# mklarqvist/libflagstats

Measured on AMD Instinct MI355X. Metric: Gflags/s + achieved HBM GB/s vs roofline, 8 GiB uint16, 1/2/4/8 MI355X, higher is better.
Workload: dtype u16; 1 GPU; 8 GiB uniform-random uint16 FLAG array (4294967296 flags) per GPU, device-resident, K1 flagstat_count accumulating into the 32 counters (atomic epilogue, one launch); flags_per_gpu=4294967296, global_flags=4294967296, parallelism=shard1, kernel_variant=71, grid_blocks=256

## Files before the change

libflagstats_amd/csrc/flagstat_capi.hip:

```cpp
#include <hip/hip_runtime.h>

#include <cstdio>
#include <cstdlib>
#include <cstring>

#include "../../include/libflagstats_hip_probe.h"
#include "flagstat_engine.h"
#include "flagstat_kernels.h"

using fsint::DeviceGuard;
using fsint::Engine;
using fsint::fail_hip;
using fsint::fail_text;

struct FLAGSTATS_hip_ctx {
    Engine* engine;
};

namespace {

#define HIP_TRY(expr)                                      \
    do {                                                   \
        hipError_t e_ = (expr);                            \
        if (e_ != hipSuccess) return fail_hip(#expr, e_);  \
// ... 121 lines not shown
        if (!fsk_variant_supported(static_cast<int>(value)))
            return fail_text("this build carries K1 schedules 9, 25 and 71 only (the sweeps' losers need make TUNING=1)");
        k.variant = static_cast<int>(value);
    } else if (!std::strcmp(key, "fuse")) {
        if (value > 1) return fail_text("fuse must be 0 or 1");
        if (value && !fsk_tuning_build())
            return fail_text("the ticket-fused finalise lost to K1 + K2 and to the atomic epilogue; it is carried by the tuning build only (make TUNING=1)");
        k.fuse = static_cast<int>(value);
    } else if (!std::strcmp(key, "anatomy")) {
        if (!fsk_tuning_build()) return fail_text("anatomy is a tuning-build knob (make TUNING=1)");
        fsk_set_anatomy(static_cast<int>(value));
    } else if (!std::strcmp(key, "epilogue")) {
        if (value > 1) return fail_text("epilogue must be 0 (partials + K2) or 1 (atomic adds from K1)");
        k.epilogue = static_cast<int>(value);
    } else if (!std::strcmp(key, "small_flags")) {
        k.small_flags = value;
    } else if (!std::strcmp(key, "small_bar")) {
        if (value > 1) return fail_text("small_bar must be 0 or 1");
        k.small_bar = static_cast<int>(value);
    } else if (!std::strcmp(key, "poll")) {
        if (value > 1) return fail_text("poll must be 0 or 1");
        k.poll = static_cast<int>(value);
    } else if (!std::strcmp(key, "epoch_stagger")) {
        if (value > 1) return fail_text("epoch_stagger must be 0 or 1");
        k.epoch_stagger = static_cast<int>(value);
        fsk_set_epoch_stagger(k.epoch_stagger.load());
    } else if (!std::strcmp(key, "group_min_grid")) {
        if (value > 0xFFFFFFFFull) return fail_text("group_min_grid must fit 32 bits");
        k.group_min_grid = static_cast<uint32_t>(value);
        fsk_set_group_min_grid(k.group_min_grid.load());
    } else if (!std::strcmp(key, "group_max_steps")) {
        k.group_max_steps = value;
        fsk_set_group_max_steps(value);
    } else if (!std::strcmp(key, "dyn_lg_queues")) {
        if (value > 4) return fail_text("dyn_lg_queues must be 0..4");
        k.dyn_lgq = static_cast<uint32_t>(value);
        if (fsk_tuning_build()) fsk_set_dyn_queues(k.dyn_lgq.load());
    } else if (!std::strcmp(key, "dyn_first_pct") || !std::strcmp(key, "dyn_div") || !std::strcmp(key, "dyn_cmax") ||
               !std::strcmp(key, "dyn_min_steps")) {
        std::atomic<uint32_t>& slot = key[4] == 'f' ? k.dyn_first_pct : key[4] == 'd' ? k.dyn_div : key[4] == 'c' ? k.dyn_cmax : k.dyn_min_steps;
        if ((key[4] == 'f' && value > 100) || (key[4] == 'd' && (value < 1 || value > 64)) || (key[4] == 'c' && (value < 1 || value > 65535)) ||
            value > 0xFFFFFFFFull)
            return fail_text("dyn_first_pct 0..100, dyn_div 1..64, dyn_cmax 1..65535");
        slot = static_cast<uint32_t>(value);
        if (fsk_tuning_build()) fsk_set_dyn(k.dyn_first_pct.load(), k.dyn_div.load(), k.dyn_cmax.load(), k.dyn_min_steps.load());
    } else if (!std::strcmp(key, "chunk_flags")) {
        if (value < 8) return fail_text("chunk_flags must be >= 8");
        k.chunk_flags = value;
    } else if (!std::strcmp(key, "on_error")) {
        if (value > 1) return fail_text("on_error must be 0 (return) or 1 (abort)");
        k.on_error = static_cast<int>(value);
    } else if (!std::strcmp(key, "fence_free_events")) {
        if (value > 1) return fail_text("fence_free_events must be 0 or 1");
        k.fence_free_events = static_cast<int>(value);
    } else if (!std::strcmp(key, "lz4_decoder")) {
        if (value > 2) return fail_text("lz4_decoder must be 0 (host threads), 1 (GPU) or 2 (by file size)");
        k.lz4_decoder = static_cast<int>(value);
    } else if (!std::strcmp(key, "zstd_decoder")) {
        if (value > 2) return fail_text("zstd_decoder must be 0 (libzstd on host threads), 1 (GPU) or 2 (by file size)");
        k.zstd_decoder = static_cast<int>(value);
    } else if (!std::strcmp(key, "zstd_gpu_min_bytes")) {
        k.zstd_gpu_min_bytes = value;
    } else if (!std::strcmp(key, "lz4_gpu_kernel")) {
        if (value > 1) return fail_text("lz4_gpu_kernel must be 0 (workgroup pipeline) or 1 (one wave per block)");
        k.lz4_gpu_kernel = static_cast<int>(value);
    } else if (!std::strcmp(key, "lz4_gpu_min_bytes")) {
        k.lz4_gpu_min_bytes = value;
    } else if (!std::strcmp(key, "staged_min_flags")) {
        k.staged_min_flags = value;
    } else if (!std::strcmp(key, "lz4_gpu_keep_bytes")) {
        k.lz4_gpu_keep_bytes = value;
    } else if (!std::strcmp(key, "numa")) {
        if (value > 1) return fail_text("numa must be 0 or 1");
        k.numa = static_cast<int>(value);
    } else {
        return fail_text("unknown key");
    }
    return 0;
}

uint64_t FLAGSTATS_hip_get(const char* key)
{
    if (fsint::process_guard(__func__)) return 0;
    if (!key) return 0;
    fsint::Knobs& k = fsint::knobs();
    if (!std::strcmp(key, "blocks_per_cu")) return k.blocks_per_cu ? k.blocks_per_cu.load() : 1;
    if (!std::strcmp(key, "variant")) return static_cast<uint64_t>(k.variant.load());
    if (!std::strcmp(key, "chunk_flags")) return k.chunk_flags.load();
    if (!std::strcmp(key, "dyn_first_pct")) return k.dyn_first_pct.load();
    if (!std::strcmp(key, "dyn_div")) return k.dyn_div.load();
    if (!std::strcmp(key, "dyn_cmax")) return k.dyn_cmax.load();
    if (!std::strcmp(key, "dyn_min_steps")) return k.dyn_min_steps.load();
    if (!std::strcmp(key, "dyn_lg_queues")) return k.dyn_lgq.load();
    if (!std::strcmp(key, "group_min_grid")) return k.group_min_grid.load();
    if (!std::strcmp(key, "group_max_steps")) return k.group_max_steps.load();
    if (!std::strcmp(key, "last_k1_two_level")) return (fsk_last_mode() >> 3) & 1;
    if (!std::strcmp(key, "small_flags")) return k.small_flags.load();
    if (!std::strcmp(key, "small_bar")) return static_cast<uint64_t>(k.small_bar.load());
    if (!std::strcmp(key, "small_in_is_device")) {
        if (fsint::default_device() < 0) return 0;
        Engine* e = fsint::default_engine();
        return e && e->small_bar_in ? 1 : 0;
    }
    if (!std::strcmp(key, "poll")) return static_cast<uint64_t>(k.poll.load());
    if (!std::strcmp(key, "epoch_stagger")) return static_cast<uint64_t>(k.epoch_stagger.load());
    if (!std::strcmp(key, "fuse")) return static_cast<uint64_t>(k.fuse.load());
    if (!std::strcmp(key, "epilogue")) return static_cast<uint64_t>(k.epilogue.load());
    if (!std::strcmp(key, "tuning_build")) return static_cast<uint64_t>(fsk_tuning_build());
    if (!std::strcmp(key, "on_error")) return static_cast<uint64_t>(k.on_error.load());
    if (!std::strcmp(key, "numa")) return static_cast<uint64_t>(k.numa.load());
    if (!std::strcmp(key, "lz4_decoder")) return static_cast<uint64_t>(k.lz4_decoder.load());
    if (!std::strcmp(key, "zstd_decoder")) return static_cast<uint64_t>(k.zstd_decoder.load());
    if (!std::strcmp(key, "zstd_gpu_min_bytes")) return k.zstd_gpu_min_bytes.load();
    if (!std::strcmp(key, "lz4_gpu_kernel")) return static_cast<uint64_t>(k.lz4_gpu_kernel.load());
    if (!std::strcmp(key, "lz4_gpu_min_bytes")) return k.lz4_gpu_min_bytes.load();
    if (!std::strcmp(key, "staged_min_flags")) return k.staged_min_flags.load();
    if (!std::strcmp(key, "staged_calls")) return k.staged_calls.load();
    if (!std::strcmp(key, "lz4_gpu_keep_bytes")) return k.lz4_gpu_keep_bytes.load();
    if (!std::strcmp(key, "lz4_gpu_kept_bytes")) {
        if (fsint::default_device() < 0) return 0;
        Engine* e = fsint::default_engine();
        if (!e) return 0;
        std::lock_guard<std::mutex> lk(e->mu);
        uint64_t held = e->lz4_cap[0] + e->lz4_cap[1];
        for (uint64_t c : e->zstd_scratch_cap) held += c;
        return held;
    }
    if (!std::strcmp(key, "user_workspaces")) {
        if (fsint::default_device() < 0) return 0;
// ... 467 lines not shown
```

libflagstats_amd/csrc/flagstat_count_core.h:

```cpp
#ifndef FLAGSTAT_COUNT_CORE_H_
#define FLAGSTAT_COUNT_CORE_H_

#include <hip/hip_runtime.h>
#include <stdint.h>

#include "flagstat_device.h"
#include "flagstat_kernels.h"

namespace fsk {

__device__ __forceinline__ void front4(uint32_t L, uint32_t H, uint32_t& T, uint32_t& selq, uint32_t& keep)
{
    const uint32_t sel1 = (L >> 1) & 0x07070707u;
    const uint32_t abc = perm(0x09091B19u, 0x09092B29u, sel1);
    const uint32_t m = __builtin_amdgcn_bitop3_b32(L, abc, 0xC4C4C4C4u, 0xE4);

    const uint32_t h1 = H >> 1;
    const uint32_t idx = and_or(h1, 0x04040404u, lshl1_or(L & 0x01010101u, H & 0x01010101u));
    keep = perm(0x050C050Cu, 0x05F60504u, idx);
    T = m & keep;

    selq = h1 & 0x03030303u;
}

// ... 161 lines not shown
        if constexpr (ATOMIC) {
            if (add) (void)__hip_atomic_fetch_add(&out[threadIdx.x], add, __ATOMIC_RELAXED, __HIP_MEMORY_SCOPE_AGENT);
        } else {
            if (mode & 1)
                out[threadIdx.x] = add;
            else if (add)
                out[threadIdx.x] += add;
        }
    }
}

__device__ __forceinline__ void grouped_epilogue(const uint64_t* tot, uint64_t* __restrict__ out, int mode, uint64_t n_flags,
                                                 uint64_t* __restrict__ block)
{
    if (threadIdx.x >= 64) return;
    const uint32_t g = blockIdx.x & 7u;
    const uint32_t members = (gridDim.x - g + 7u) >> 3;
    uint64_t* copy = block + kGroupCopyWord + 32 * g;
    uint64_t* ticket = block + kGroupTicketWord + 16 * g;
    const uint64_t add = threadIdx.x < 32 ? slot_value(tot, mode, n_flags) : 0;
    if (add) (void)__hip_atomic_fetch_add(&copy[threadIdx.x], add, __ATOMIC_RELAXED, __HIP_MEMORY_SCOPE_AGENT);
    asm volatile("s_waitcnt vmcnt(0)" ::: "memory");
    uint32_t t = 0;
    if (threadIdx.x == 0) t = static_cast<uint32_t>(__hip_atomic_fetch_add(ticket, 1ull, __ATOMIC_RELAXED, __HIP_MEMORY_SCOPE_AGENT));
    t = __builtin_amdgcn_readfirstlane(t);
    if (t != members - 1) return;
    if (threadIdx.x < 32) {
        const uint64_t v = __hip_atomic_exchange(&copy[threadIdx.x], 0ull, __ATOMIC_RELAXED, __HIP_MEMORY_SCOPE_AGENT);
        if (v) (void)__hip_atomic_fetch_add(&out[threadIdx.x], v, __ATOMIC_RELAXED, __HIP_MEMORY_SCOPE_AGENT);
    }
    if (threadIdx.x == 0) __hip_atomic_store(ticket, 0ull, __ATOMIC_RELAXED, __HIP_MEMORY_SCOPE_AGENT);
}

template <bool NT, int USTRIDE, int VPS = kVecPerStep>
__device__ __forceinline__ void load_step(uint4 (&v)[kUnroll], const uint4* __restrict__ a0, uint64_t st, uint64_t lane_off,
                                          uint64_t lo, uint64_t hi, uint64_t fast_begin, uint64_t fast_end)
{
    const uint64_t j0 = st * VPS + lane_off;
    if (st >= fast_begin && st < fast_end) {
#pragma unroll
        for (int u = 0; u < kUnroll; ++u) v[u] = load_vec<NT>(a0 + j0 + u * USTRIDE);
    } else {
#pragma unroll
        for (int u = 0; u < kUnroll; ++u) v[u] = load_guarded(a0, j0 + u * USTRIDE, lo, hi);
    }
}

}

#endif
```

libflagstats_amd/csrc/flagstat_engine.h:

```cpp
#ifndef FLAGSTAT_ENGINE_H_
#define FLAGSTAT_ENGINE_H_

#include <hip/hip_runtime.h>
#include <stdint.h>

#include <sched.h>

#include <atomic>
#include <cstdio>
#include <condition_variable>
#include <functional>
#include <list>
#include <memory>
#include <mutex>
#include <thread>
#include <utility>
#include <vector>

struct FLAGSTATS_gpu_lz4_stats;

namespace fsint {

struct Workspace {
    uint64_t* partials = nullptr;
    uint32_t grid_cap = 0;
};

struct Knobs {
    std::atomic<uint32_t> blocks_per_cu{0};
    std::atomic<int> variant{71};
    std::atomic<uint32_t> dyn_first_pct{75}, dyn_div{4}, dyn_cmax{32}, dyn_min_steps{32}, dyn_lgq{3};
    std::atomic<uint64_t> small_flags{1ull << 20};
    std::atomic<int> small_bar{1};
    std::atomic<int> poll{1};
    std::atomic<int> epoch_stagger{1};
    std::atomic<uint32_t> group_min_grid{64};
    std::atomic<uint64_t> group_max_steps{40};
    std::atomic<int> fuse{0};
    std::atomic<int> epilogue{1};
    std::atomic<uint64_t> chunk_flags{32ull << 20};
    std::atomic<int> on_error{1};
    std::atomic<int> lz4_decoder{2};
    std::atomic<int> lz4_gpu_kernel{0};
    std::atomic<uint64_t> lz4_gpu_min_bytes{64ull << 20};
    std::atomic<uint64_t> staged_min_flags{1ull << 27};
    std::atomic<uint64_t> staged_calls{0};
    std::atomic<uint64_t> lz4_gpu_keep_bytes{~0ull};
    std::atomic<int> zstd_decoder{2};
    std::atomic<uint64_t> zstd_gpu_min_bytes{64ull << 20};
    std::atomic<int> fence_free_events{0};
    std::atomic<int> numa{1};
};
Knobs& knobs();

enum { OP_FLAGSTAT = 0, OP_POSPOPCNT = 1, OP_FLAGSTAT_STORE = 2, OP_BASE_MASK = 3, OP_SUPERSET = 4, OP_HOST_OUT = 8 };

struct RegisteredHost {
    void* ptr = nullptr;
    void* map = nullptr;
    size_t map_bytes = 0;
    size_t len = 0;
    bool registered = false;
    bool refused = false;
};

class WorkerPool {
  public:
    WorkerPool() = default;
    ~WorkerPool();
    WorkerPool(const WorkerPool&) = delete;
    WorkerPool& operator=(const WorkerPool&) = delete;
    bool start(int n, std::function<void(int)> fn);
    void wait();
    int threads() const { return static_cast<int>(threads_.size()); }

  private:
    void loop(int id, uint64_t born);
    std::mutex m_;
    std::condition_variable cv_job_, cv_done_;
    std::vector<std::thread> threads_;
    std::function<void(int)> job_;
    uint64_t generation_ = 0;
    int want_ = 0, running_ = 0;
    bool stop_ = false;
};

// ... 180 lines not shown
```

libflagstats_amd/csrc/flagstat_engine.hip:

```cpp
#include "flagstat_engine.h"

#include <emmintrin.h>
#include <smmintrin.h>
#include <sys/syscall.h>
#include <pthread.h>
#include <sys/mman.h>
#include <unistd.h>

#include <cstdio>
#include <cstdlib>
#include <chrono>
#include <cstring>
#include <memory>
#include <string>
#include <thread>
#include <vector>

#include "flagstat_kernels.h"

namespace fsint {

namespace {

constexpr size_t kHostOutBytes = 1024;
// ... 28 lines not shown
        }
        if (have == 0xFFFFFFFFu) return 0;
        _mm_pause();
    }
    return 1;
}

uint64_t env_u64(const char* name, uint64_t dflt)
{
    const char* s = std::getenv(name);
    if (!s || !*s) return dflt;
    return std::strtoull(s, nullptr, 0);
}

void read_env_knobs()
{
    std::call_once(g_env_once, [] {
        g_knobs.blocks_per_cu = static_cast<uint32_t>(env_u64("FLAGSTATS_HIP_BLOCKS_PER_CU", g_knobs.blocks_per_cu));
        g_knobs.variant = static_cast<int>(env_u64("FLAGSTATS_HIP_VARIANT", static_cast<uint64_t>(g_knobs.variant)));
        g_knobs.chunk_flags = env_u64("FLAGSTATS_HIP_CHUNK_FLAGS", g_knobs.chunk_flags);
        g_knobs.dyn_first_pct = static_cast<uint32_t>(env_u64("FLAGSTATS_HIP_DYN_FIRST_PCT", g_knobs.dyn_first_pct));
        g_knobs.dyn_div = static_cast<uint32_t>(env_u64("FLAGSTATS_HIP_DYN_DIV", g_knobs.dyn_div));
        g_knobs.dyn_cmax = static_cast<uint32_t>(env_u64("FLAGSTATS_HIP_DYN_CMAX", g_knobs.dyn_cmax));
        g_knobs.dyn_min_steps = static_cast<uint32_t>(env_u64("FLAGSTATS_HIP_DYN_MIN_STEPS", g_knobs.dyn_min_steps));
        g_knobs.small_flags = env_u64("FLAGSTATS_HIP_SMALL_FLAGS", g_knobs.small_flags);
        g_knobs.small_bar = static_cast<int>(env_u64("FLAGSTATS_HIP_SMALL_BAR", static_cast<uint64_t>(g_knobs.small_bar)));
        g_knobs.poll = static_cast<int>(env_u64("FLAGSTATS_HIP_POLL", static_cast<uint64_t>(g_knobs.poll)));
        g_knobs.epoch_stagger = static_cast<int>(env_u64("FLAGSTATS_HIP_EPOCH_STAGGER", static_cast<uint64_t>(g_knobs.epoch_stagger)));
        fsk_set_epoch_stagger(g_knobs.epoch_stagger.load());
        g_knobs.group_min_grid = static_cast<uint32_t>(env_u64("FLAGSTATS_HIP_GROUP_MIN_GRID", g_knobs.group_min_grid));
        fsk_set_group_min_grid(g_knobs.group_min_grid.load());
        g_knobs.group_max_steps = env_u64("FLAGSTATS_HIP_GROUP_MAX_STEPS", g_knobs.group_max_steps);
        fsk_set_group_max_steps(g_knobs.group_max_steps.load());
        g_knobs.dyn_lgq = static_cast<uint32_t>(env_u64("FLAGSTATS_HIP_DYN_LG_QUEUES", g_knobs.dyn_lgq));
        if (fsk_tuning_build()) {
            fsk_set_dyn_queues(g_knobs.dyn_lgq.load());
            fsk_set_dyn(g_knobs.dyn_first_pct.load(), g_knobs.dyn_div.load(), g_knobs.dyn_cmax.load(), g_knobs.dyn_min_steps.load());
        }
        g_knobs.fuse = fsk_tuning_build() ? static_cast<int>(env_u64("FLAGSTATS_HIP_FUSE", static_cast<uint64_t>(g_knobs.fuse))) : 0;
        g_knobs.epilogue = static_cast<int>(env_u64("FLAGSTATS_HIP_EPILOGUE", static_cast<uint64_t>(g_knobs.epilogue)));
        g_knobs.numa = static_cast<int>(env_u64("FLAGSTATS_HIP_NUMA", static_cast<uint64_t>(g_knobs.numa)));
        g_knobs.fence_free_events = static_cast<int>(env_u64("FLAGSTATS_HIP_FENCE_FREE_EVENTS", static_cast<uint64_t>(g_knobs.fence_free_events)));
        g_knobs.lz4_decoder = static_cast<int>(env_u64("FLAGSTATS_HIP_LZ4_DECODER", static_cast<uint64_t>(g_knobs.lz4_decoder)));
        g_knobs.lz4_gpu_kernel = static_cast<int>(env_u64("FLAGSTATS_HIP_LZ4_GPU_KERNEL", static_cast<uint64_t>(g_knobs.lz4_gpu_kernel)));
        g_knobs.lz4_gpu_min_bytes = env_u64("FLAGSTATS_HIP_LZ4_GPU_MIN_BYTES", g_knobs.lz4_gpu_min_bytes);
        g_knobs.staged_min_flags = env_u64("FLAGSTATS_HIP_STAGED_MIN_FLAGS", g_knobs.staged_min_flags);
        g_knobs.zstd_decoder = static_cast<int>(env_u64("FLAGSTATS_HIP_ZSTD_DECODER", static_cast<uint64_t>(g_knobs.zstd_decoder)));
        if (g_knobs.zstd_decoder > 2) g_knobs.zstd_decoder = 2;
        g_knobs.zstd_gpu_min_bytes = env_u64("FLAGSTATS_HIP_ZSTD_GPU_MIN_BYTES", g_knobs.zstd_gpu_min_bytes);
        g_knobs.lz4_gpu_keep_bytes = env_u64("FLAGSTATS_HIP_LZ4_GPU_KEEP_BYTES", g_knobs.lz4_gpu_keep_bytes);
        const char* oe = std::getenv("FLAGSTATS_HIP_ON_ERROR");
        if (oe && *oe) g_knobs.on_error = (!std::strcmp(oe, "return") || !std::strcmp(oe, "0")) ? 0 : 1;
    });
}

#define HIP_TRY(expr)                                      \
    do {                                                   \
        hipError_t e_ = (expr);                            \
        if (e_ != hipSuccess) return fail_hip(#expr, e_);  \
    } while (0)

int numa_node_of_device(int device)
{
    char bus[64] = {0};
    if (hipDeviceGetPCIBusId(bus, sizeof bus, device) != hipSuccess) return -1;
    for (char* p = bus; *p; ++p)
// ... 232 lines not shown
        std::lock_guard<std::mutex> lk(m_);
        job_ = std::move(fn);
        want_ = n;
        running_ = n;
        ++generation_;
    }
    cv_job_.notify_all();
    return true;
}

void WorkerPool::wait()
{
    {
        std::unique_lock<std::mutex> ul(m_);
        cv_done_.wait(ul, [&] { return running_ == 0; });
        want_ = 0;
    }
    static const bool per_call = [] {
        const char* k = std::getenv("FLAGSTATS_HIP_POOL");
        return k && std::atoi(k) == 0;
    }();
    if (per_call) {
        {
            std::lock_guard<std::mutex> lk(m_);
            stop_ = true;
        }
        cv_job_.notify_all();
        for (std::thread& t : threads_) t.join();
        threads_.clear();
        stop_ = false;
    }
}

Knobs& knobs()
{
    if (!g_forked.load(std::memory_order_relaxed)) read_env_knobs();
    return g_knobs;
}

bool process_forked()
{
    if (g_forked.load(std::memory_order_relaxed)) return true;
    const pid_t owner = g_owner_pid.load(std::memory_order_relaxed);
    if (owner != 0 && owner != getpid()) {
        g_forked.store(true, std::memory_order_relaxed);
        return true;
    }
    return false;
}

int process_guard(const char* entry, bool quiet)
{
    if (!g_forked.load(std::memory_order_relaxed)) {
        const pid_t me = getpid();
        pid_t owner = g_owner_pid.load(std::memory_order_acquire);
        if (owner == me) return 0;
        if (owner == 0) {
            if (g_owner_pid.compare_exchange_strong(owner, me, std::memory_order_acq_rel)) {
                (void)pthread_atfork(nullptr, nullptr, mark_forked_child);
                read_env_knobs();
                return 0;
            }
            if (owner == me) return 0;
        }
        g_forked.store(true, std::memory_order_relaxed);
    }
// ... 694 lines not shown
```

libflagstats_amd/csrc/flagstat_kernels.h:

```cpp
#ifndef FLAGSTAT_KERNELS_H_
#define FLAGSTAT_KERNELS_H_

#include <hip/hip_runtime.h>
#include <stddef.h>
#include <stdint.h>

namespace fsk {

constexpr int kThreads = 256;
constexpr int kUnroll = 8;
constexpr int kVecPerStep = kThreads * kUnroll;
constexpr int kGroupTicketWord = 288;
constexpr int kGroupCopyWord = 512;
constexpr int kInternal = 21;

struct DynSched {
    uint64_t* block;
    uint32_t c0;
    uint32_t inv;
    uint32_t cmax;
    uint32_t lgq;
};

struct HostSignal {
    uint64_t* pairs;
    uint64_t value;
};

struct CountArgs {
    const void* a0;
    uint64_t lo, hi;
    uint64_t nsteps;
    uint64_t fast_begin;
    uint64_t fast_end;
    uint32_t grid;
    uint64_t* partials;
    uint32_t* ticket;
    uint64_t* out;
    DynSched dyn;
    HostSignal sig;
    int mode;
};

}

extern "C" {
size_t fsk_partials_bytes(uint32_t grid);
void fsk_warm(void);
hipError_t fsk_launch(const uint16_t* d_array, uint64_t n, uint32_t grid, int variant, uint64_t* d_partials,
                      uint32_t* d_ticket, uint64_t* d_out32, hipStream_t stream, uint64_t* signal_word = nullptr,
                      uint64_t signal_value = 0);
int fsk_variant_supported(int variant);
void fsk_set_dyn(uint32_t first_pct, uint32_t div, uint32_t cmax, uint32_t min_steps_per_wg) __attribute__((weak));
void fsk_set_dyn_queues(uint32_t lg_queues) __attribute__((weak));
void fsk_set_anatomy(int bits) __attribute__((weak));
void fsk_launch_policy(int* stagger, uint32_t* group_min_grid, uint64_t* group_max_steps);
void fsk_note_mode(int mode);
hipError_t fsk_launch_finalize(uint64_t* d_partials, uint32_t grid, uint64_t* d_out32, int mode, uint64_t n, fsk::HostSignal sig,
                               hipStream_t stream);
void fsk_set_group_min_grid(uint32_t min_grid);
void fsk_set_group_max_steps(uint64_t max_steps_per_workgroup);
int fsk_last_mode(void);
void fsk_set_epoch_stagger(int on);
int fsk_tuning_build(void);
hipError_t fsk_launch_pospopcnt(const uint16_t* d_array, uint64_t n, uint32_t grid, uint64_t* d_partials,
                                uint64_t* d_out16, hipStream_t stream, int direct);
hipError_t fsk_clock_probe(uint64_t* d_out, uint32_t grid, uint64_t ticks, hipStream_t stream);
hipError_t fsk_generate(uint16_t* d_array, uint64_t n, int kind, uint64_t seed, uint32_t mask, uint64_t first_index,
                        hipStream_t stream);
}

#endif
```

libflagstats_amd/csrc/flagstat_kernels.hip:

```cpp
#include <hip/hip_runtime.h>
#include <stdint.h>

#include <atomic>

#include "flagstat_count_core.h"

namespace fsk {

template <int DEPTH, int STAGE, bool NT, int USTRIDE, bool HAS_NEXT = true>
__device__ __forceinline__ void step(Lane<DEPTH>& s, uint4 (&v)[kUnroll], uint32_t blk, const uint4* __restrict__ next,
                                     const uint4* __restrict__ cur = nullptr)
{
    static_assert(STAGE == 0 || STAGE == 1 || STAGE == 9, "the product carries three schedules; the others: flagstat_kernels_tuning.hip");
    uint32_t t8a = 0, t8b = 0, f8a = 0, f8b = 0, s8a = 0, s8b = 0;
#pragma unroll
    for (int half = 0; half < 2; ++half) {
        uint32_t t4a = 0, t4b = 0, f4a = 0, f4b = 0, s4a = 0, s4b = 0;
#pragma unroll
        for (int q = 0; q < 2; ++q) {
            uint32_t T[4], F[4], S[4];
#pragma unroll
            for (int k = 0; k < 2; ++k) {
                uint32_t L0, H0, L1, H1;
                const int uu = half * 4 + q * 2 + k;
// ... 38 lines not shown
            csa(q ? s4b : s4a, s.s2, s.s2, s2a, s2b);
        }
        csa(half ? t8b : t8a, s.t4, s.t4, t4a, t4b);
        csa(half ? f8b : f8a, s.f4, s.f4, f4a, f4b);
        csa(half ? s8b : s8a, s.s4, s.s4, s4a, s4b);
    }
    uint32_t ct, cf, cs;
    csa(ct, s.t8, s.t8, t8a, t8b);
    csa(cf, s.f8, s.f8, f8a, f8b);
    csa(cs, s.s8, s.s8, s8a, s8b);
    chain_push<0, DEPTH>(s, blk, ct, cf, cs);
}

template <int DEPTH, int STAGE = 0, bool NT = false, int USTRIDE = 64, bool HAS_NEXT = true>
__device__ __forceinline__ void step_and_count(Lane<DEPTH>& s, uint4 (&v)[kUnroll], uint32_t& blk,
                                               const uint4* __restrict__ next = nullptr, const uint4* __restrict__ cur = nullptr)
{
    blk = __builtin_amdgcn_readfirstlane(blk);
    step<DEPTH, STAGE, NT, USTRIDE, HAS_NEXT>(s, v, blk, next, cur);
    ++blk;
    if (blk == (1u << DEPTH) - 1u) {
        flush(s, (1u << DEPTH) - 1u);
        blk = 0;
    }
}

template <int DEPTH, bool NT, bool PREFETCH, bool INTERLEAVE, int STAGE>
__global__ __launch_bounds__(kThreads) void flagstat_count(const uint4* __restrict__ a0, uint64_t lo, uint64_t hi,
                                                           uint64_t nsteps, uint64_t fast_begin, uint64_t fast_end,
                                                           uint64_t* __restrict__ partials, uint32_t* ticket,
                                                           uint64_t* out, int mode, DynSched dyn, HostSignal sig)
{
    static_assert(!PREFETCH, "the two-register-buffer loop lives in flagstat_kernels_tuning.hip");
    Lane<DEPTH> s;
    lane_init(s);
    const uint32_t lane = threadIdx.x & 63u;
    const uint32_t wave = threadIdx.x >> 6;
    constexpr int T = kThreads;
    constexpr int VPS = T * kUnroll;
    constexpr int US = INTERLEAVE ? T : 64;
    const uint64_t lane_off = INTERLEAVE ? static_cast<uint64_t>(threadIdx.x)
                                         : static_cast<uint64_t>(wave) * (64 * kUnroll) + lane;
    const uint64_t G = gridDim.x;
    uint32_t blk = (mode & 16) ? (wave & 3u) * 64u : 0u;

    constexpr bool ROLL = (STAGE != 0);
    if constexpr (ROLL) {
        if (fast_begin != 0 && blockIdx.x == 0 && wave < T / 64) {
            uint4 v[kUnroll];
            load_step<NT, US, VPS>(v, a0, 0, lane_off, lo, hi, fast_begin, fast_end);
            step_and_count(s, v, blk);
        }
        if (nsteps > fast_end && nsteps - 1 >= fast_begin && (nsteps - 1) % G == blockIdx.x && wave < T / 64) {
            uint4 v[kUnroll];
            load_step<NT, US, VPS>(v, a0, nsteps - 1, lane_off, lo, hi, fast_begin, fast_end);
            step_and_count(s, v, blk);
        }
        uint64_t st = blockIdx.x;
        if (st < fast_begin) st += G;
        if constexpr (STAGE == 1) {
            if (st < fast_end) {
                uint4 v[kUnroll];
                const uint4* p = a0 + st * kVecPerStep + lane_off;
#pragma unroll
                for (int u = 0; u < kUnroll; ++u) {
                    v[u] = load_vec<NT>(p + u * US);
                    __builtin_amdgcn_sched_barrier(0);
                }
                for (; st + G < fast_end; st += G) {
                    p += G * kVecPerStep;
                    step_and_count<DEPTH, STAGE, NT, US>(s, v, blk, p);
                }
                step_and_count(s, v, blk);
            }
        } else {
            constexpr int RD = 6;
            if (st < fast_end) {
                uint4 v[kUnroll];
                const uint4* p = a0 + st * VPS + lane_off;
#pragma unroll
                for (int u = 0; u < RD; ++u) {
                    v[u] = load_vec<NT>(p + u * US);
                    __builtin_amdgcn_sched_barrier(0);
                }
                for (; st + G < fast_end; st += G) {
                    const uint4* pn = p + G * VPS;
                    step_and_count<DEPTH, STAGE, NT, US, true>(s, v, blk, pn, p);
                    p = pn;
                }
                step_and_count<DEPTH, STAGE, NT, US, false>(s, v, blk, nullptr, p);
            }
        }
    } else {
        for (uint64_t st = blockIdx.x; st < nsteps; st += G) {
            uint4 v[kUnroll];
            load_step<NT, US>(v, a0, st, lane_off, lo, hi, fast_begin, fast_end);
            step_and_count(s, v, blk);
        }
    }
    flush(s, blk);

    constexpr int kWaves = kThreads / 64;
    __shared__ uint32_t red[kWaves][kInternal];
    uint32_t wsum[kInternal];
#pragma unroll
    for (int c = 0; c < kInternal; ++c) wsum[c] = wave_sum_lane63(s.acc[c]);
    if (lane == 63 && wave < kWaves) {
// ... 47 lines not shown
    }
    __syncthreads();
    if (sig.pairs != nullptr) {
        if (threadIdx.x < 32) store_pair(sig, slot_value(tot, mode, n_flags));
        return;
    }
    finalize_slots(tot, out, mode, n_flags);
}

}

extern "C" hipError_t fsk_tuning_launch(const uint16_t* d_array, uint64_t n, uint32_t grid, int variant, uint64_t* d_partials,
                                        uint32_t* d_ticket, uint64_t* d_out32, hipStream_t stream, uint64_t* signal_word,
                                        uint64_t signal_value) __attribute__((weak));
extern "C" int fsk_tuning_variant_supported(int variant) __attribute__((weak));

extern "C" void fsk_warm(void)
{
    hipFuncAttributes attr;
    if (hipFuncGetAttributes(&attr, reinterpret_cast<const void*>(&fsk::flagstat_finalize)) != hipSuccess) (void)hipGetLastError();
}

extern "C" size_t fsk_partials_bytes(uint32_t grid) { return static_cast<size_t>(grid) * fsk::kInternal * sizeof(uint64_t) + 8192; }

static std::atomic<int> g_epoch_stagger{1};

extern "C" void fsk_set_epoch_stagger(int on) { g_epoch_stagger = on ? 1 : 0; }

static std::atomic<uint32_t> g_group_min_grid{64};
static std::atomic<uint64_t> g_group_max_steps{40};

extern "C" void fsk_set_group_min_grid(uint32_t min_grid) { g_group_min_grid = min_grid; }
extern "C" void fsk_set_group_max_steps(uint64_t max_steps) { g_group_max_steps = max_steps; }

static std::atomic<int> g_last_mode{0};
extern "C" int fsk_last_mode(void) { return g_last_mode.load(); }

extern "C" void fsk_launch_policy(int* stagger, uint32_t* group_min_grid, uint64_t* group_max_steps)
{
    *stagger = g_epoch_stagger.load();
    *group_min_grid = g_group_min_grid.load();
    *group_max_steps = g_group_max_steps.load();
}
extern "C" void fsk_note_mode(int mode) { g_last_mode.store(mode, std::memory_order_relaxed); }

extern "C" hipError_t fsk_launch_finalize(uint64_t* d_partials, uint32_t grid, uint64_t* d_out32, int mode, uint64_t n, fsk::HostSignal sig,
                                          hipStream_t stream)
{
    hipLaunchKernelGGL(fsk::flagstat_finalize, dim3(1), dim3(fsk::kFinalizeThreads), 0, stream, d_partials, grid, d_out32, mode, n, sig);
    return hipGetLastError();
}

template <int DEPTH, bool NT, bool PREFETCH, bool INTERLEAVE, int STAGE = 0>
static hipError_t launch_count_t(const fsk::CountArgs& a, hipStream_t stream)
{
    hipLaunchKernelGGL((fsk::flagstat_count<DEPTH, NT, PREFETCH, INTERLEAVE, STAGE>), dim3(a.grid), dim3(fsk::kThreads), 0, stream,
                       reinterpret_cast<const uint4*>(a.a0), a.lo, a.hi, a.nsteps, a.fast_begin, a.fast_end, a.partials,
                       a.ticket, a.out, a.mode, a.dyn, a.sig);
    return hipGetLastError();
}

extern "C" hipError_t fsk_launch(const uint16_t* d_array, uint64_t n, uint32_t grid, int variant, uint64_t* d_partials,
                                 uint32_t* d_ticket, uint64_t* d_out32, hipStream_t stream, uint64_t* signal_word,
                                 uint64_t signal_value)
{
    if (fsk_tuning_launch)
        return fsk_tuning_launch(d_array, n, grid, variant, d_partials, d_ticket, d_out32, stream, signal_word, signal_value);
    if (n == 0) return hipSuccess;
    if (grid == 0 || d_array == nullptr || d_partials == nullptr || d_out32 == nullptr) return hipErrorInvalidValue;
    const uintptr_t addr = reinterpret_cast<uintptr_t>(d_array);
    if (addr & 1u) return hipErrorInvalidValue;
    fsk::CountArgs a;
    const uintptr_t base = addr & ~static_cast<uintptr_t>(15);
    a.a0 = reinterpret_cast<const void*>(base);
    a.lo = (addr - base) / 2;
    a.hi = a.lo + n;
    const uint64_t nvec = (a.hi + 7) / 8;
    const uint64_t vps = fsk::kVecPerStep;
    a.nsteps = (nvec + vps - 1) / vps;
    a.fast_begin = (a.lo == 0) ? 0 : 1;
    a.fast_end = (a.hi / 8) / vps;
    if (a.fast_end < a.fast_begin) a.fast_end = a.fast_begin;
    if (static_cast<uint64_t>(grid) > a.nsteps) grid = static_cast<uint32_t>(a.nsteps);
    a.grid = grid;
    a.partials = d_partials;
    a.mode = ((variant >> 8) & 1) | (((variant >> 10) & 1) << 1) | (((variant >> 11) & 1) << 2);
    if ((a.mode & 4) && (a.mode & 1)) return hipErrorInvalidValue;
    if ((variant >> 9) & 1) return hipErrorInvalidValue;
    a.ticket = nullptr;
    a.out = d_out32;
    a.dyn = fsk::DynSched{reinterpret_cast<uint64_t*>(d_ticket), 0xFFFFFFFFu, 0, 1, 0};
    if (g_epoch_stagger.load()) a.mode |= 16;
    a.sig = fsk::HostSignal{signal_word, signal_value};
    if (signal_word && !(a.mode & 1)) return hipErrorInvalidValue;
    if (signal_word && (a.mode & 1) && !(a.mode & 4) && grid == 1) a.mode |= 32;
    if ((a.mode & 4) && grid >= g_group_min_grid.load() && (a.nsteps + grid - 1) / grid <= g_group_max_steps.load() && d_ticket != nullptr)
        a.mode |= 8;
    g_last_mode.store(a.mode, std::memory_order_relaxed);
    hipError_t e;
    switch (variant & 255) {
    case 9: e = launch_count_t<8, true, false, true>(a, stream); break;
    case 25: e = launch_count_t<8, true, false, true, 1>(a, stream); break;
    case 71: e = launch_count_t<8, true, false, false, 9>(a, stream); break;
    default: return hipErrorInvalidValue;
    }
    if (e != hipSuccess) return e;
    if (a.mode & (4 | 32)) return hipSuccess;
    return fsk_launch_finalize(d_partials, grid, d_out32, a.mode, n, a.sig, stream);
}

extern "C" int fsk_variant_supported(int variant)
{
    switch (variant & 255) {
    case 9:
    case 25:
    case 71: return 1;
    default: return fsk_tuning_variant_supported ? fsk_tuning_variant_supported(variant) : 0;
    }
}

extern "C" int fsk_tuning_build(void) { return fsk_tuning_launch ? 1 : 0; }
```

libflagstats_amd/csrc/flagstat_kernels_tuning.hip:

```cpp
#include <hip/hip_runtime.h>
#include <stdint.h>

#include <atomic>

#include "flagstat_count_core.h"

namespace fskt {
using namespace fsk;

struct LdsStage {
    const uint4* lane;
    uint32_t slot0;
    uint32_t first;
};

template <bool NT>
__device__ __forceinline__ void lds_dma16(const uint4* gsrc, uint32_t lds_dst)
{
    uint32_t keep;
    const uint32_t dst = __builtin_amdgcn_readfirstlane(lds_dst);
    if constexpr (NT)
        asm volatile("s_mov_b32 %0, m0\n\ts_mov_b32 m0, %2\n\ts_nop 0\n\tglobal_load_lds_dwordx4 %1, off nt\n\ts_mov_b32 m0, %0"
                     : "=&s"(keep) : "v"(gsrc), "s"(dst) : "memory");
    else
// ... 177 lines not shown
                const uint4* p = a0 + st * kVecPerStep + lane_off;
#pragma unroll
                for (int u = 0; u < kUnroll; ++u) {
                    v[u] = load_vec<NT>(p + u * US);
                    __builtin_amdgcn_sched_barrier(0);
                }
                for (; st + G < fast_end; st += G) {
                    p += G * kVecPerStep;
                    step_and_count<DEPTH, STAGE, NT, US>(s, v, blk, p);
                    FSK_TL_ONCE(1);
                }
                step_and_count(s, v, blk);
                FSK_TL_ONCE(1);
            }
        } else if constexpr (STAGE == 5 || STAGE == 9 || STAGE == 10 || STAGE == 11 || STAGE == 12) {
            constexpr int RD = STAGE == 5 ? 4 : ((STAGE == 9 || STAGE == 12) ? 6 : (STAGE == 10 ? 7 : 5));
            if (st < fast_end) {
                uint4 v[kUnroll];
                const uint4* p = a0 + st * VPS + lane_off;
#pragma unroll
                for (int u = 0; u < RD; ++u) {
                    v[u] = load_vec<NT>(p + u * US);
                    __builtin_amdgcn_sched_barrier(0);
                }
                for (; st + G < fast_end; st += G) {
                    const uint4* pn = p + G * VPS;
                    step_and_count<DEPTH, STAGE, NT, US, true>(s, v, blk, pn, LdsStage{nullptr, 0, 0}, p);
                    FSK_TL_ONCE(1);
                    p = pn;
                }
                step_and_count<DEPTH, STAGE, NT, US, false>(s, v, blk, nullptr, LdsStage{nullptr, 0, 0}, p);
                FSK_TL_ONCE(1);
            }
        } else if constexpr (STAGE == 13 || STAGE == 14) {
            if (wave & 1u)
                roll_partial<DEPTH, STAGE == 13 ? 10 : 11, NT, US, VPS>(s, blk, a0, st, G, fast_end, lane_off);
            else
                roll_partial<DEPTH, 9, NT, US, VPS>(s, blk, a0, st, G, fast_end, lane_off);
        } else if constexpr (STAGE == 4) {
            const uint64_t N = fast_end - fast_begin;
            const uint64_t c0 = dyn.c0;
            const uint64_t D0 = G * c0;
            const bool dynamic = N > D0;
            __shared__ uint64_t tix[4];
            if (wave == kThreads / 64) {
                if (dynamic) {
                    const uint32_t lgq = dyn.lgq;
                    const uint64_t M = N - D0;
                    const uint32_t qi = (blockIdx.x >> 3) & ((1u << lgq) - 1u);
                    const uint64_t qb = D0 + ((M * qi) >> lgq), qe = D0 + ((M * (qi + 1)) >> lgq);
                    uint64_t* ctr = dyn.block + 16 * (qi + 1);
                    uint64_t start[4] = {0, 0, 0, 0};
                    uint64_t pos = qb;
                    auto grab = [&](uint32_t k) {
                        const uint64_t rem = pos < qe ? qe - pos : 0;
                        const uint32_t r32 = rem > 0xFFFFFFFFull ? 0xFFFFFFFFu : static_cast<uint32_t>(rem);
                        uint32_t c = __umulhi(r32, dyn.inv);
                        c = c < 1u ? 1u : c;
                        c = c > dyn.cmax ? dyn.cmax : c;
                        uint64_t r = 0;
                        if (lane == 0) r = __hip_atomic_fetch_add(ctr, static_cast<uint64_t>(c), __ATOMIC_RELAXED, __HIP_MEMORY_SCOPE_AGENT);
                        const uint32_t rl = __builtin_amdgcn_readfirstlane(static_cast<uint32_t>(r));
                        const uint32_t rh = __builtin_amdgcn_readfirstlane(static_cast<uint32_t>(r >> 32));
                        uint64_t st = qb + ((static_cast<uint64_t>(rh) << 32) | rl);
                        uint64_t len = c;
                        if (st >= qe) {
// ... 305 lines not shown
    if (g_timeline && (a.mode & 4)) {
        a.mode |= 2048;
        a.ticket = reinterpret_cast<uint32_t*>(g_timeline);
    }
    a.out = d_out32;
    a.dyn = fsk::DynSched{reinterpret_cast<uint64_t*>(d_ticket), 0xFFFFFFFFu, 0, 1, 0};
    if (stagger) a.mode |= 16;
    a.sig = fsk::HostSignal{signal_word, signal_value};
    if (signal_word && !(a.mode & 1)) return hipErrorInvalidValue;
    if (signal_word && (a.mode & 1) && !(a.mode & 4) && grid == 1 && !((variant >> 9) & 1)) a.mode |= 32;
    if ((a.mode & 4) && grid >= group_min_grid && (a.nsteps + grid - 1) / grid <= group_max_steps &&
        d_ticket != nullptr && !(a.mode & 4096))
        a.mode |= 8;
    if (variant & 128) {
        const uint64_t full = a.fast_end - a.fast_begin;
        const uint64_t per_wg = (full + grid - 1) / grid;
        uint64_t c0 = per_wg;
        if (per_wg >= g_dyn_min_steps.load() && per_wg >= 2) {
            c0 = full * g_dyn_first_pct.load() / (100ull * grid);
            if (c0 < 1) c0 = 1;
        }
        if (c0 > 0xFFFFFFFFull) c0 = 0xFFFFFFFFull;
        uint32_t lgq = g_dyn_lgq.load();
        while (lgq && (grid >> (3 + lgq)) == 0) --lgq;
        uint64_t per_queue = (static_cast<uint64_t>(grid) >> lgq) * g_dyn_div.load();
        if (per_queue < 2) per_queue = 2;
        a.dyn.block = reinterpret_cast<uint64_t*>(d_ticket);
        a.dyn.c0 = static_cast<uint32_t>(c0);
        a.dyn.inv = static_cast<uint32_t>((1ull << 32) / per_queue);
        a.dyn.cmax = g_dyn_cmax.load();
        a.dyn.lgq = lgq;
    }
    if (((variant >> 9) & 1) && d_ticket == nullptr) return hipErrorInvalidValue;
    fsk_note_mode(a.mode);
    hipError_t e;
    switch (variant & 255) {
    case 9: e = launch_count_t<8, true, false, true>(a, stream); break;
    case 25: e = launch_count_t<8, true, false, true, 1>(a, stream); break;
    case 71: e = launch_count_t<8, true, false, false, 9>(a, stream); break;
    case 153: e = launch_count_t<8, true, false, true, 4>(a, stream); break;
    case 29: e = launch_count_t<8, true, false, true, 5>(a, stream); break;
    case 57: e = launch_count_t<8, true, false, true, 6>(a, stream); break;
    case 17: e = launch_count_t<8, true, false, false, 1>(a, stream); break;
    case 61: e = launch_count_t<8, true, false, true, 7>(a, stream); break;
    case 63: e = launch_count_t<8, true, false, true, 8>(a, stream); break;
    case 65: e = launch_count_t<8, true, false, true, 11>(a, stream); break;
    case 67: e = launch_count_t<8, true, false, true, 9>(a, stream); break;
    case 69: e = launch_count_t<8, true, false, true, 10>(a, stream); break;
    case 73: e = launch_count_t<8, true, false, true, 12>(a, stream); break;
    case 75: e = launch_count_t<8, true, false, false, 11>(a, stream); break;
    case 79: e = launch_count_t<8, true, false, false, 13>(a, stream); break;
    case 81: e = launch_count_t<8, true, false, false, 14>(a, stream); break;
    case 77: e = launch_count_t<8, true, false, false, 10>(a, stream); break;
    case 0: e = launch_count_t<8, false, false, false>(a, stream); break;
    case 1: e = launch_count_t<8, true, false, false>(a, stream); break;
    case 13: e = launch_count_t<8, true, true, true>(a, stream); break;
    case 27: e = launch_count_t<7, true, false, true, 1>(a, stream); break;
    case 41: e = launch_count_t<8, true, false, true, 2>(a, stream); break;
    case 89: e = launch_count_t<8, true, false, true, 3>(a, stream); break;
    default: return hipErrorInvalidValue;
    }
    if (e != hipSuccess) return e;
    if (a.ticket || (a.mode & (4 | 32))) return hipSuccess;
    return fsk_launch_finalize(d_partials, grid, d_out32, a.mode, n, a.sig, stream);
}

extern "C" void fsk_set_anatomy(int bits) { g_anatomy = bits; }

extern "C" uint32_t fsk_timeline_run(const uint16_t* d_array, uint64_t n, uint32_t grid, int variant, int warm,
                                     uint64_t* h_rows, uint32_t cap_rows)
{
    if (grid == 0 || grid > cap_rows) return 0;
// ... 74 lines not shown
```

Before: 3684 Gflags/s.

## Add dynamic ticket-claimed tail to static-stride count kernel variant 71

For variant 71, the last few percent of the input (default 2%) are taken out of the static grid-stride schedule and handed out as small contiguous chunks. Waves claim these chunks through per-queue atomic tickets, with a configurable claim-ahead distance. The aim is to remove end-of-kernel load imbalance, where some workgroups finish their static share late and leave CUs idle. In exchange it adds atomic traffic on ticket counters and a counter reset by the wave that draws the last ticket. It also brings new tuning knobs and environment variables.

```diff
diff --git a/libflagstats_amd/csrc/flagstat_capi.hip b/libflagstats_amd/csrc/flagstat_capi.hip
--- a/libflagstats_amd/csrc/flagstat_capi.hip
+++ b/libflagstats_amd/csrc/flagstat_capi.hip
@@ -177,6 +177,23 @@
     } else if (!std::strcmp(key, "group_max_steps")) {
         k.group_max_steps = value;
         fsk_set_group_max_steps(value);
+    } else if (!std::strcmp(key, "tail_pct") || !std::strcmp(key, "tail_min_steps") || !std::strcmp(key, "tail_max_steps") ||
+               !std::strcmp(key, "tail_min_grid") || !std::strcmp(key, "tail_lg_queues")) {
+        if (!std::strcmp(key, "tail_pct")) {
+            if (value > 100) return fail_text("tail_pct must be 0 (off) .. 100");
+            k.tail_pct = static_cast<uint32_t>(value);
+        } else if (!std::strcmp(key, "tail_min_steps")) {
+            k.tail_min_steps = value;
+        } else if (!std::strcmp(key, "tail_max_steps")) {
+            k.tail_max_steps = value;
+        } else if (!std::strcmp(key, "tail_min_grid")) {
+            if (value > 0xFFFFFFFFull) return fail_text("tail_min_grid must fit 32 bits");
+            k.tail_min_grid = static_cast<uint32_t>(value);
+        } else {
+            if (value > 4) return fail_text("tail_lg_queues must be 0..4");
+            k.tail_lg_queues = static_cast<uint32_t>(value);
+        }
+        fsint::push_tail_policy();
     } else if (!std::strcmp(key, "dyn_lg_queues")) {
         if (value > 4) return fail_text("dyn_lg_queues must be 0..4");
         k.dyn_lgq = static_cast<uint32_t>(value);
@@ -240,6 +257,12 @@
     if (!std::strcmp(key, "group_min_grid")) return k.group_min_grid.load();
     if (!std::strcmp(key, "group_max_steps")) return k.group_max_steps.load();
     if (!std::strcmp(key, "last_k1_two_level")) return (fsk_last_mode() >> 3) & 1;
+    if (!std::strcmp(key, "tail_pct")) return k.tail_pct.load();
+    if (!std::strcmp(key, "tail_min_steps")) return k.tail_min_steps.load();
+    if (!std::strcmp(key, "tail_max_steps")) return k.tail_max_steps.load();
+    if (!std::strcmp(key, "tail_min_grid")) return k.tail_min_grid.load();
+    if (!std::strcmp(key, "tail_lg_queues")) return k.tail_lg_queues.load();
+    if (!std::strcmp(key, "last_k1_tail")) return (fsk_last_mode() >> 6) & 1;
     if (!std::strcmp(key, "small_flags")) return k.small_flags.load();
     if (!std::strcmp(key, "small_bar")) return static_cast<uint64_t>(k.small_bar.load());
     if (!std::strcmp(key, "small_in_is_device")) {
diff --git a/libflagstats_amd/csrc/flagstat_count_core.h b/libflagstats_amd/csrc/flagstat_count_core.h
--- a/libflagstats_amd/csrc/flagstat_count_core.h
+++ b/libflagstats_amd/csrc/flagstat_count_core.h
@@ -217,6 +217,81 @@
     if (threadIdx.x == 0) __hip_atomic_store(ticket, 0ull, __ATOMIC_RELAXED, __HIP_MEMORY_SCOPE_AGENT);
 }
 
+template <int D>
+struct TailClaim {
+    uint32_t* ctr;
+    uint32_t q, lgq;
+    uint32_t L;
+    uint32_t last;
+    bool closes;
+    uint32_t tk[D];
+};
+
+template <int D>
+__device__ __forceinline__ void tail_setup(TailClaim<D>& tc, uint64_t* __restrict__ block, uint32_t lgq, uint32_t chunks, uint32_t wave)
+{
+    const uint32_t Q = 1u << lgq;
+    const uint32_t G = gridDim.x;
+    const uint32_t qv = (wave + 4u * (blockIdx.x >> 3)) & (Q - 1u);
+    const uint32_t q = __builtin_amdgcn_readfirstlane(qv);
+    uint32_t W;
+    if (lgq < 2) {
+        W = G << (2 - lgq);
+    } else {
+        const uint32_t lgr = lgq - 2, R = 1u << lgr, k = q >> 2;
+        const uint32_t full = G >> 3, rem = G & 7u;
+        W = 8u * ((full + R - 1u - k) >> lgr) + (((full & (R - 1u)) == k) ? rem : 0u);
+    }
+    tc.q = q;
+    tc.lgq = lgq;
+    tc.L = chunks > q ? (chunks - q + Q - 1u) >> lgq : 0u;
+    tc.last = tc.L + static_cast<uint32_t>(D) * W - 1u;
+    tc.ctr = reinterpret_cast<uint32_t*>(block + kTailTicketWord + 16u * qv);
+    tc.closes = false;
+#pragma unroll
+    for (int i = 0; i < D; ++i) tc.tk[i] = 0;
+}
+
+template <int D>
+__device__ __forceinline__ uint32_t tail_draw(const TailClaim<D>& tc)
+{
+    uint32_t t = 0;
+    if ((threadIdx.x & 63u) == 0) t = __hip_atomic_fetch_add(tc.ctr, 1u, __ATOMIC_RELAXED, __HIP_MEMORY_SCOPE_AGENT);
+    return t;
+}
+
+template <int D>
+__device__ __forceinline__ void tail_start(TailClaim<D>& tc)
+{
+#pragma unroll
+    for (int i = 0; i < D; ++i) tc.tk[i] = tail_draw(tc);
+}
+
+template <int D>
+__device__ __forceinline__ uint32_t tail_take(TailClaim<D>& tc)
+{
+    const uint32_t t = __builtin_amdgcn_readfirstlane(tc.tk[0]);
+    tc.closes |= t == tc.last;
+#pragma unroll
+    for (int i = 0; i + 1 < D; ++i) tc.tk[i] = tc.tk[i + 1];
+    if (t < tc.L) tc.tk[D - 1] = tail_draw(tc);
+    return t;
+}
+
+template <int D>
+__device__ __forceinline__ void tail_finish(TailClaim<D>& tc)
+{
+#pragma unroll
+    for (int i = 0; i + 1 < D; ++i) tc.closes |= __builtin_amdgcn_readfirstlane(tc.tk[i]) == tc.last;
+    if (tc.closes && (threadIdx.x & 63u) == 0) __hip_atomic_store(tc.ctr, 0u, __ATOMIC_RELAXED, __HIP_MEMORY_SCOPE_AGENT);
+}
+
+template <int D>
+__device__ __forceinline__ uint64_t tail_chunk_vec(const TailClaim<D>& tc, uint32_t t)
+{
+    return ((static_cast<uint64_t>(t) << tc.lgq) + tc.q) * (64u * kUnroll);
+}
+
 template <bool NT, int USTRIDE, int VPS = kVecPerStep>
 __device__ __forceinline__ void load_step(uint4 (&v)[kUnroll], const uint4* __restrict__ a0, uint64_t st, uint64_t lane_off,
                                           uint64_t lo, uint64_t hi, uint64_t fast_begin, uint64_t fast_end)
diff --git a/libflagstats_amd/csrc/flagstat_engine.h b/libflagstats_amd/csrc/flagstat_engine.h
--- a/libflagstats_amd/csrc/flagstat_engine.h
+++ b/libflagstats_amd/csrc/flagstat_engine.h
@@ -36,6 +36,8 @@
     std::atomic<int> epoch_stagger{1};
     std::atomic<uint32_t> group_min_grid{64};
     std::atomic<uint64_t> group_max_steps{40};
+    std::atomic<uint32_t> tail_pct{2}, tail_min_grid{64}, tail_lg_queues{4};
+    std::atomic<uint64_t> tail_min_steps{384}, tail_max_steps{~0ull};
     std::atomic<int> fuse{0};
     std::atomic<int> epilogue{1};
     std::atomic<uint64_t> chunk_flags{32ull << 20};
@@ -52,6 +54,7 @@
     std::atomic<int> numa{1};
 };
 Knobs& knobs();
+void push_tail_policy();
 
 enum { OP_FLAGSTAT = 0, OP_POSPOPCNT = 1, OP_FLAGSTAT_STORE = 2, OP_BASE_MASK = 3, OP_SUPERSET = 4, OP_HOST_OUT = 8 };
 
diff --git a/libflagstats_amd/csrc/flagstat_engine.hip b/libflagstats_amd/csrc/flagstat_engine.hip
--- a/libflagstats_amd/csrc/flagstat_engine.hip
+++ b/libflagstats_amd/csrc/flagstat_engine.hip
@@ -84,6 +84,14 @@
         fsk_set_group_min_grid(g_knobs.group_min_grid.load());
         g_knobs.group_max_steps = env_u64("FLAGSTATS_HIP_GROUP_MAX_STEPS", g_knobs.group_max_steps);
         fsk_set_group_max_steps(g_knobs.group_max_steps.load());
+        g_knobs.tail_pct = static_cast<uint32_t>(env_u64("FLAGSTATS_HIP_TAIL_PCT", g_knobs.tail_pct));
+        g_knobs.tail_min_steps = env_u64("FLAGSTATS_HIP_TAIL_MIN_STEPS", g_knobs.tail_min_steps);
+        g_knobs.tail_max_steps = env_u64("FLAGSTATS_HIP_TAIL_MAX_STEPS", g_knobs.tail_max_steps);
+        g_knobs.tail_min_grid = static_cast<uint32_t>(env_u64("FLAGSTATS_HIP_TAIL_MIN_GRID", g_knobs.tail_min_grid));
+        g_knobs.tail_lg_queues = static_cast<uint32_t>(env_u64("FLAGSTATS_HIP_TAIL_LG_QUEUES", g_knobs.tail_lg_queues));
+        if (fsk_set_tail_policy)
+            fsk_set_tail_policy(g_knobs.tail_pct.load(), g_knobs.tail_min_steps.load(), g_knobs.tail_max_steps.load(),
+                                g_knobs.tail_min_grid.load(), g_knobs.tail_lg_queues.load());
         g_knobs.dyn_lgq = static_cast<uint32_t>(env_u64("FLAGSTATS_HIP_DYN_LG_QUEUES", g_knobs.dyn_lgq));
         if (fsk_tuning_build()) {
             fsk_set_dyn_queues(g_knobs.dyn_lgq.load());
@@ -382,6 +390,13 @@
     }
 }
 
+void push_tail_policy()
+{
+    if (fsk_set_tail_policy)
+        fsk_set_tail_policy(g_knobs.tail_pct.load(), g_knobs.tail_min_steps.load(), g_knobs.tail_max_steps.load(), g_knobs.tail_min_grid.load(),
+                            g_knobs.tail_lg_queues.load());
+}
+
 Knobs& knobs()
 {
     if (!g_forked.load(std::memory_order_relaxed)) read_env_knobs();
diff --git a/libflagstats_amd/csrc/flagstat_kernels.h b/libflagstats_amd/csrc/flagstat_kernels.h
--- a/libflagstats_amd/csrc/flagstat_kernels.h
+++ b/libflagstats_amd/csrc/flagstat_kernels.h
@@ -12,6 +12,11 @@
 constexpr int kVecPerStep = kThreads * kUnroll;
 constexpr int kGroupTicketWord = 288;
 constexpr int kGroupCopyWord = 512;
+constexpr int kTailTicketWord = 768;
+#ifndef FSK_TAIL_DISTANCE
+#define FSK_TAIL_DISTANCE 1
+#endif
+constexpr int kTailDistance = FSK_TAIL_DISTANCE;
 constexpr int kInternal = 21;
 
 struct DynSched {
@@ -60,6 +65,8 @@
                                hipStream_t stream);
 void fsk_set_group_min_grid(uint32_t min_grid);
 void fsk_set_group_max_steps(uint64_t max_steps_per_workgroup);
+void fsk_set_tail_policy(uint32_t pct, uint64_t min_steps, uint64_t max_steps, uint32_t min_grid, uint32_t lg_queues) __attribute__((weak));
+bool fsk_tail_plan(fsk::CountArgs* a, int variant, const uint32_t* d_ticket);
 int fsk_last_mode(void);
 void fsk_set_epoch_stagger(int on);
 int fsk_tuning_build(void);
diff --git a/libflagstats_amd/csrc/flagstat_kernels.hip b/libflagstats_amd/csrc/flagstat_kernels.hip
--- a/libflagstats_amd/csrc/flagstat_kernels.hip
+++ b/libflagstats_amd/csrc/flagstat_kernels.hip
@@ -94,6 +94,7 @@
                                                            uint64_t* out, int mode, DynSched dyn, HostSignal sig)
 {
     static_assert(!PREFETCH, "the two-register-buffer loop lives in flagstat_kernels_tuning.hip");
+    static_assert(STAGE != 10 || !INTERLEAVE, "a ticket names a contiguous 8 KiB");
     Lane<DEPTH> s;
     lane_init(s);
     const uint32_t lane = threadIdx.x & 63u;
@@ -135,6 +136,54 @@
                 }
                 step_and_count(s, v, blk);
             }
+        } else if constexpr (STAGE == 10) {
+            constexpr int RD = 6;
+            constexpr int D = kTailDistance;
+            const uint64_t static_end = dyn.c0;
+            TailClaim<D> tc;
+            tail_setup(tc, dyn.block, dyn.lgq, dyn.cmax, wave);
+            const uint4* tail0 = a0 + (static_end > fast_begin ? static_end : fast_begin) * VPS + lane;
+            uint4 v[kUnroll];
+            const uint4* p = nullptr;
+            bool have = st < static_end;
+            if (have) {
+                p = a0 + st * VPS + lane_off;
+                if (st + G >= static_end) tail_start(tc);
+#pragma unroll
+                for (int u = 0; u < RD; ++u) {
+                    v[u] = load_vec<NT>(p + u * US);
+                    __builtin_amdgcn_sched_barrier(0);
+                }
+                for (; st + G < static_end; st += G) {
+                    if (st + 2 * G >= static_end) tail_start(tc);
+                    const uint4* pn = p + G * VPS;
+                    step_and_count<DEPTH, 9, NT, US, true>(s, v, blk, pn, p);
+                    p = pn;
+                }
+            } else {
+                tail_start(tc);
+                const uint32_t t = tail_take(tc);
+                have = t < tc.L;
+                if (have) {
+                    p = tail0 + tail_chunk_vec(tc, t);
+#pragma unroll
+                    for (int u = 0; u < RD; ++u) {
+                        v[u] = load_vec<NT>(p + u * US);
+                        __builtin_amdgcn_sched_barrier(0);
+                    }
+                }
+            }
+            if (have) {
+                uint32_t t = tail_take(tc);
+                while (t < tc.L) {
+                    const uint4* pn = tail0 + tail_chunk_vec(tc, t);
+                    step_and_count<DEPTH, 9, NT, US, true>(s, v, blk, pn, p);
+                    p = pn;
+                    t = tail_take(tc);
+                }
+                step_and_count<DEPTH, 9, NT, US, false>(s, v, blk, nullptr, p);
+            }
+            tail_finish(tc);
         } else {
             constexpr int RD = 6;
             if (st < fast_end) {
@@ -248,6 +297,45 @@
 
 extern "C" void fsk_set_group_min_grid(uint32_t min_grid) { g_group_min_grid = min_grid; }
 extern "C" void fsk_set_group_max_steps(uint64_t max_steps) { g_group_max_steps = max_steps; }
+
+static std::atomic<uint32_t> g_tail_pct{2};
+static std::atomic<uint64_t> g_tail_min_steps{384};
+static std::atomic<uint64_t> g_tail_max_steps{~0ull};
+static std::atomic<uint32_t> g_tail_min_grid{64};
+static std::atomic<uint32_t> g_tail_lgq{4};
+
+extern "C" void fsk_set_tail_policy(uint32_t pct, uint64_t min_steps, uint64_t max_steps, uint32_t min_grid, uint32_t lg_queues)
+{
+    g_tail_pct = pct > 100 ? 100 : pct;
+    g_tail_min_steps = min_steps;
+    g_tail_max_steps = max_steps;
+    g_tail_min_grid = min_grid;
+    g_tail_lgq = lg_queues > 4 ? 4 : lg_queues;
+}
+
+extern "C" bool fsk_tail_plan(fsk::CountArgs* a, int variant, const uint32_t* d_ticket)
+{
+    const uint32_t pct = g_tail_pct.load();
+    const uint64_t per_wg = (a->nsteps + a->grid - 1) / a->grid;
+    if ((variant & 255) != 71 || pct == 0 || d_ticket == nullptr || (a->mode & 32) || a->grid < g_tail_min_grid.load() ||
+        per_wg < g_tail_min_steps.load() || per_wg > g_tail_max_steps.load())
+        return false;
+    const uint64_t full = a->fast_end - a->fast_begin;
+    const uint64_t tail = (full * pct + 99) / 100;
+    uint64_t static_end = (a->fast_end - tail) / a->grid * a->grid;
+    if (static_end < a->fast_begin) static_end = 0;
+    const uint64_t tail_begin = static_end > a->fast_begin ? static_end : a->fast_begin;
+    const uint64_t chunks = 4 * (a->fast_end - tail_begin);
+    if (static_end > 0xFFFFFFFFull || chunks > 0x7FFFFFFFull) return false;
+    a->dyn.c0 = static_cast<uint32_t>(static_end);
+    a->dyn.inv = 0;
+    a->dyn.cmax = static_cast<uint32_t>(chunks);
+    uint32_t lgq = g_tail_lgq.load();
+    while (lgq > 2 && ((a->grid + 7) >> 3) < (1u << (lgq - 2))) --lgq;
+    a->dyn.lgq = lgq;
+    a->mode |= 64;
+    return true;
+}
 
 static std::atomic<int> g_last_mode{0};
 extern "C" int fsk_last_mode(void) { return g_last_mode.load(); }
@@ -312,12 +400,14 @@
     if (signal_word && (a.mode & 1) && !(a.mode & 4) && grid == 1) a.mode |= 32;
     if ((a.mode & 4) && grid >= g_group_min_grid.load() && (a.nsteps + grid - 1) / grid <= g_group_max_steps.load() && d_ticket != nullptr)
         a.mode |= 8;
+    const bool tail = fsk_tail_plan(&a, variant, d_ticket);
     g_last_mode.store(a.mode, std::memory_order_relaxed);
     hipError_t e;
-    switch (variant & 255) {
+    switch (tail ? 256 : (variant & 255)) {
     case 9: e = launch_count_t<8, true, false, true>(a, stream); break;
     case 25: e = launch_count_t<8, true, false, true, 1>(a, stream); break;
     case 71: e = launch_count_t<8, true, false, false, 9>(a, stream); break;
+    case 256: e = launch_count_t<8, true, false, false, 10>(a, stream); break;
     default: return hipErrorInvalidValue;
     }
     if (e != hipSuccess) return e;
diff --git a/libflagstats_amd/csrc/flagstat_kernels_tuning.hip b/libflagstats_amd/csrc/flagstat_kernels_tuning.hip
--- a/libflagstats_amd/csrc/flagstat_kernels_tuning.hip
+++ b/libflagstats_amd/csrc/flagstat_kernels_tuning.hip
@@ -233,6 +233,58 @@
                 step_and_count<DEPTH, STAGE, NT, US, false>(s, v, blk, nullptr, LdsStage{nullptr, 0, 0}, p);
                 FSK_TL_ONCE(1);
             }
+        } else if constexpr (STAGE == 15) {
+            constexpr int RD = 6;
+            constexpr int D = kTailDistance;
+            const uint64_t static_end = dyn.c0;
+            TailClaim<D> tc;
+            tail_setup(tc, dyn.block, dyn.lgq, dyn.cmax, wave);
+            const uint4* tail0 = a0 + (static_end > fast_begin ? static_end : fast_begin) * VPS + lane;
+            const LdsStage none{nullptr, 0, 0};
+            uint4 v[kUnroll];
+            const uint4* p = nullptr;
+            bool have = st < static_end;
+            if (have) {
+                p = a0 + st * VPS + lane_off;
+                if (st + G >= static_end) tail_start(tc);
+#pragma unroll
+                for (int u = 0; u < RD; ++u) {
+                    v[u] = load_vec<NT>(p + u * US);
+                    __builtin_amdgcn_sched_barrier(0);
+                }
+                for (; st + G < static_end; st += G) {
+                    if (st + 2 * G >= static_end) tail_start(tc);
+                    const uint4* pn = p + G * VPS;
+                    step_and_count<DEPTH, 9, NT, US, true>(s, v, blk, pn, none, p);
+                    FSK_TL_ONCE(1);
+                    p = pn;
+                }
+            } else {
+                tail_start(tc);
+                const uint32_t t = tail_take(tc);
+                have = t < tc.L;
+                if (have) {
+                    p = tail0 + tail_chunk_vec(tc, t);
+#pragma unroll
+                    for (int u = 0; u < RD; ++u) {
+                        v[u] = load_vec<NT>(p + u * US);
+                        __builtin_amdgcn_sched_barrier(0);
+                    }
+                }
+            }
+            if (have) {
+                uint32_t t = tail_take(tc);
+                while (t < tc.L) {
+                    const uint4* pn = tail0 + tail_chunk_vec(tc, t);
+                    step_and_count<DEPTH, 9, NT, US, true>(s, v, blk, pn, none, p);
+                    FSK_TL_ONCE(1);
+                    p = pn;
+                    t = tail_take(tc);
+                }
+                step_and_count<DEPTH, 9, NT, US, false>(s, v, blk, nullptr, none, p);
+                FSK_TL_ONCE(1);
+            }
+            tail_finish(tc);
         } else if constexpr (STAGE == 13 || STAGE == 14) {
             if (wave & 1u)
                 roll_partial<DEPTH, STAGE == 13 ? 10 : 11, NT, US, VPS>(s, blk, a0, st, G, fast_end, lane_off);
@@ -604,12 +656,13 @@
         a.dyn.lgq = lgq;
     }
     if (((variant >> 9) & 1) && d_ticket == nullptr) return hipErrorInvalidValue;
+    const bool tail = !(a.mode & 4096) && !(g_anatomy & 1) && fsk_tail_plan(&a, variant, d_ticket);
     fsk_note_mode(a.mode);
     hipError_t e;
     switch (variant & 255) {
     case 9: e = launch_count_t<8, true, false, true>(a, stream); break;
     case 25: e = launch_count_t<8, true, false, true, 1>(a, stream); break;
-    case 71: e = launch_count_t<8, true, false, false, 9>(a, stream); break;
+    case 71: e = !tail ? launch_count_t<8, true, false, false, 9>(a, stream) : launch_count_t<8, true, false, false, 15>(a, stream); break;
     case 153: e = launch_count_t<8, true, false, true, 4>(a, stream); break;
     case 29: e = launch_count_t<8, true, false, true, 5>(a, stream); break;
     case 57: e = launch_count_t<8, true, false, true, 6>(a, stream); break;
```

Measured after the change: 3692 Gflags/s (median of 6 runs). No clear change (+0.2%).
